# seung-lab/euclidean-distance-transform-3d

Hardware: NVIDIA B200
Metric: Mvoxels/s edtsq 512^3 uint32 (higher is better)
Workload: dtype f32 (u32 labels)

## Files before the change

euclidean-distance-transform-3d_b200/csrc/edt_capi.cu:

```cuda
#include "edt_host.h"
#include "edt_voxel_graph.cuh"
#include "edt_each.cuh"
#include "edt_slab.cuh"

#include <cstdarg>
#include <cstdio>
#include <cstdlib>
#include <cstring>
#include <dlfcn.h>
#include <condition_variable>
#include <functional>
#include <mutex>
#include <thread>
#include <vector>

namespace edtb200 {
namespace host {

thread_local char g_error[512] = "";

int fail(int code, const char* fmt, ...) {
  va_list ap;
  va_start(ap, fmt);
  vsnprintf(g_error, sizeof(g_error), fmt, ap);
// ... 343 lines not shown
    return launch_first<decltype(lw)::Bytes>(labels, f, nlines, sx, wx, border, kflags, dc, s);
  });
}

int later_pass(int axis, int label_bytes, const void* labels, float* f, int64_t sx, int64_t sy, int64_t sz,
               int64_t part, const float* w, int border_lo, int border_hi, int kflags, bool pdl, DeviceCache& dc,
               cudaStream_t s) {
  const int64_t n[2] = {sx, sy};
  const edtb200::LineGeom g = axis == 1 ? geom_for_axis(1, sx, sy, part) : geom_for_axis(2, sx, part, sz);
  return with_label_width(label_bytes, [&](auto lw) {
    return launch_later<decltype(lw)::Bytes>(labels, f, g, w[axis], border_lo, border_hi, kflags, dc, s, pdl,
                                             integer_bound(w, n, axis));
  });
}

template <class T>
cudaError_t grow(T*& p, size_t& have, size_t need) {
  if (have >= need) return cudaSuccess;
  if (p) cudaFree(p);
  p = nullptr; have = 0;
  const cudaError_t e = cudaMalloc(&p, need);
  if (e == cudaSuccess) have = need;
  return e;
}

cudaError_t ensure_stream(cudaStream_t& s) {
  return s ? cudaSuccess : cudaStreamCreateWithFlags(&s, cudaStreamNonBlocking);
}

constexpr int kProfileRing = 256;
thread_local bool g_profile = false;
thread_local cudaEvent_t g_pass_events[kProfileRing][4];
thread_local bool g_pass_events_init = false;
thread_local int g_pass_marks[kProfileRing];
thread_local long g_pass_seq = 0;

void mark_pass(int idx, cudaStream_t stream) {
  if (!g_profile) return;
  if (!g_pass_events_init) {
    for (auto& slot : g_pass_events) for (auto& e : slot) e = nullptr;
    g_pass_events_init = true;
  }
  if (idx == 0) ++g_pass_seq;
  const int slot = (int)((g_pass_seq - 1) % kProfileRing);
  cudaEvent_t& e = g_pass_events[slot][idx];
  if (!e && cudaEventCreate(&e) != cudaSuccess) { cudaGetLastError(); return; }
  cudaEventRecord(e, stream);
  g_pass_marks[slot] = idx;
}

typedef int (*NvtxPushFn)(const char*);
typedef int (*NvtxPopFn)(void);
NvtxPushFn g_nvtx_push = nullptr;
NvtxPopFn g_nvtx_pop = nullptr;
std::once_flag g_nvtx_once;

void nvtx_init() {
  std::call_once(g_nvtx_once, [] {
    if (getenv("EDTB200_NO_NVTX")) return;
    const char* names[] = {"libnvToolsExt.so.1", "libnvToolsExt.so", nullptr};
    for (int i = 0; names[i]; ++i) {
      void* h = dlopen(names[i], RTLD_NOW | RTLD_GLOBAL);
      if (!h) continue;
// ... 5 lines not shown
  });
}
void nvtx_push(const char* name) { nvtx_init(); if (g_nvtx_push) g_nvtx_push(name); }
void nvtx_pop() { if (g_nvtx_pop) g_nvtx_pop(); }

int run_passes(const void* labels, int label_bytes, int ndim, int64_t sx, int64_t sy, int64_t sz,
               float wx, float wy, float wz, int border, int flags, float* f,
               DeviceCache& dc, cudaStream_t stream) {
  const int epilogue = epilogue_flags(flags);
  const float w[3] = {wx, wy, wz};
  int rc = 0;
  static const bool verbose = getenv("EDT_B200_VERBOSE") != nullptr && atoi(getenv("EDT_B200_VERBOSE")) != 0;
  const bool profile_was = g_profile;
  if (verbose) g_profile = true;
  mark_pass(0, stream);
  nvtx_push("edt.x");
  rc = first_pass(label_bytes, labels, f, sy * sz, sx, wx, border,
                  zero_label_flags(flags) | (ndim == 1 ? epilogue : 0), dc, stream);
  nvtx_pop();
  mark_pass(1, stream);
  if (!rc && ndim >= 2) {
    nvtx_push("edt.y");
    rc = later_pass(1, label_bytes, labels, f, sx, sy, sz, sz, w, border, border, ndim == 2 ? epilogue : 0,
                    true, dc, stream);
    nvtx_pop();
    mark_pass(2, stream);
  }
  if (!rc && ndim >= 3) {
    nvtx_push("edt.z");
    rc = later_pass(2, label_bytes, labels, f, sx, sy, sz, sy, w, border, border, epilogue, true, dc,
                    stream);
    nvtx_pop();
    mark_pass(3, stream);
  }
  if (verbose) {
    g_profile = profile_was;
    float ms[3] = {0.0f, 0.0f, 0.0f};
    if (!rc && edtb200_pass_ms(0, ms) == 0) {
      const double nvox = (double)sx * (double)sy * (double)sz;
      const double total = ms[0] + ms[1] + ms[2];
      fprintf(stderr, "[edt_b200] %lldx%lldx%lld L=%d  x %.3f ms  y %.3f ms  z %.3f ms  total %.3f ms  "
                      "%.0f Mvox/s  %.0f GB/s algorithmic\n",
              (long long)sx, (long long)sy, (long long)sz, label_bytes, ms[0], ms[1], ms[2], total,
              total > 0 ? nvox / total / 1e3 : 0.0,
              total > 0 ? nvox * (3.0 * label_bytes + 20.0) / total / 1e6 : 0.0);
    }
  }
  return rc;
}


}

extern "C" {

int edtb200_version(void) { return EDTB200_VERSION; }

const char* edtb200_last_error(void) { return g_error; }
// ... 730 lines not shown
  if (p) { cudaFreeHost(p); cudaGetLastError(); }
}

int edtb200_profile_passes(int enable) {
  g_profile = enable != 0;
  if (enable) g_pass_seq = 0;
  return 0;
}

int edtb200_pass_ms(int steps_back, float* ms3) {
  if (!ms3) return fail(EDTB200_EINVAL, "null pointer");
  ms3[0] = ms3[1] = ms3[2] = 0.0f;
  if (steps_back < 0 || steps_back >= kProfileRing || steps_back >= g_pass_seq)
    return fail(EDTB200_EINVAL, "no profiled transform %d steps back", steps_back);
  const int slot = (int)((g_pass_seq - 1 - steps_back) % kProfileRing);
  for (int i = 0; i < g_pass_marks[slot] && i < 3; ++i) {
    if (!g_pass_events[slot][i] || !g_pass_events[slot][i + 1]) break;
    CUDA_TRY(cudaEventSynchronize(g_pass_events[slot][i + 1]));
    CUDA_TRY(cudaEventElapsedTime(&ms3[i], g_pass_events[slot][i], g_pass_events[slot][i + 1]));
  }
  return 0;
}

int edtb200_release(void) {
  DeviceGuard restore_device;
  int count = 0;
  if (cudaGetDeviceCount(&count) != cudaSuccess) { cudaGetLastError(); return 0; }
  for (int d = 0; d < count && d < kMaxDevices; ++d) {
    DeviceCache& dc = g_cache[d];
    std::lock_guard<std::mutex> host_call(dc.host_call);
    std::lock_guard<std::mutex> guard(dc.lock);
    if (!dc.probed) continue;
    cudaSetDevice(d);
    cudaDeviceSynchronize();
// ... 37 lines not shown
```

euclidean-distance-transform-3d_b200/csrc/edt_host.h:

```cpp
#pragma once
#include "../../include/edt_b200.h"
#include "edt_kernels.cuh"

#include <cstdint>
#include <mutex>

namespace edtb200 {
namespace host {

int fail(int code, const char* fmt, ...);

#define CUDA_TRY(expr)                                                                          \
  do {                                                                                          \
    cudaError_t e__ = (expr);                                                                   \
    if (e__ != cudaSuccess)                                                                     \
      return ::edtb200::host::fail(e__ == cudaErrorMemoryAllocation ? EDTB200_ENOMEM : EDTB200_ECUDA, \
                                   "%s failed: %s", #expr, cudaGetErrorString(e__));            \
  } while (0)

typedef CUresult (*EncodeTiledFn)(CUtensorMap*, CUtensorMapDataType, cuuint32_t, void*, const cuuint64_t*,
                                  const cuuint64_t*, const cuuint32_t*, const cuuint32_t*,
                                  CUtensorMapInterleave, CUtensorMapSwizzle, CUtensorMapL2promotion,
                                  CUtensorMapFloatOOBfill);
EncodeTiledFn tensor_map_encoder();
// ... 17 lines not shown
    cudaEvent_t ready = nullptr; cudaStream_t built_on = nullptr;
    static constexpr int kUsers = 4;
    cudaStream_t user[kUsers] = {nullptr, nullptr, nullptr, nullptr};
    cudaEvent_t used[kUsers] = {nullptr, nullptr, nullptr, nullptr};
    bool user_set[kUsers] = {false, false, false, false};
    bool many_users = false;
  };
  static constexpr int kTables = 16;
  Table tables[kTables];
  uint64_t table_clock = 0;
  cudaMemPool_t pool = nullptr;
  unsigned long long* stat_counter = nullptr;
  unsigned int* stat_ticket = nullptr;
  volatile unsigned long long* stat_publish_host = nullptr;
  unsigned long long* stat_publish_dev = nullptr;
  int sm_count = 0;
  int max_smem_optin = 0;
  bool probed = false;
};

cudaError_t scratch_alloc(DeviceCache& dc, void** p, size_t bytes, cudaStream_t stream);

int step_table(DeviceCache& dc, float w, int count, cudaStream_t stream, const float** out);
int step_table_used(DeviceCache& dc, const float* data, cudaStream_t stream);

template <int Bytes>
int launch_first(const void* labels, float* f, int64_t nlines, int64_t sx, float w, int border, int flags,
                 DeviceCache& dc, cudaStream_t stream);
template <int Bytes>
int launch_later(const void* labels, float* f, const LineGeom& g0, float w, int border_lo, int border_hi,
                 int flags, DeviceCache& dc, cudaStream_t stream, bool pdl, double fmax);

}
}
```

euclidean-distance-transform-3d_b200/csrc/edt_kernels.cuh:

```cuda
#pragma once
#include <cuda.h>
#include <cuda_runtime.h>
#include <math_constants.h>
#include <stdint.h>

namespace edtb200 {

enum : int { kSqrt = 1, kNegate = 2, kZeroLabel = 4 };

constexpr int kNoBoundary = 0x3fffffff;

template <int Bytes> struct LabelOf;
template <> struct LabelOf<1> { using type = uint8_t;  using wide = uint32_t; };
template <> struct LabelOf<2> { using type = uint16_t; using wide = uint32_t; };
template <> struct LabelOf<4> { using type = uint32_t; using wide = uint32_t; };
template <> struct LabelOf<8> { using type = uint64_t; using wide = unsigned long long; };

__device__ __forceinline__ void pdl_launch_dependents() {
  asm volatile("griddepcontrol.launch_dependents;" ::: "memory");
}
__device__ __forceinline__ void pdl_wait_for_previous_grid() {
  asm volatile("griddepcontrol.wait;" ::: "memory");
}

// ... 165 lines not shown
};
template <> struct Vec4Labels<4> {
  static __device__ __forceinline__ void load(const uint32_t* p, uint32_t v[4]) {
    const uint4 w = __ldg(reinterpret_cast<const uint4*>(p));
    v[0] = w.x; v[1] = w.y; v[2] = w.z; v[3] = w.w;
  }
};
template <> struct Vec4Labels<8> {
  static __device__ __forceinline__ void load(const uint64_t* p, unsigned long long v[4]) {
    const ulonglong2 a = __ldg(reinterpret_cast<const ulonglong2*>(p));
    const ulonglong2 b = __ldg(reinterpret_cast<const ulonglong2*>(p) + 1);
    v[0] = a.x; v[1] = a.y; v[2] = b.x; v[3] = b.y;
  }
};

template <int Bytes, int K, bool Plain>
__global__ void __launch_bounds__(256, K >= 8 ? 3 : 5)
first_axis_vec_kernel(const typename LabelOf<Bytes>::type* __restrict__ labels,
                      float* __restrict__ out, int64_t nlines, int sx,
                      const float* __restrict__ table, int border, int flags, RunStat stat) {
  using LT = typename LabelOf<Bytes>::type;
  using WT = typename LabelOf<Bytes>::wide;
  extern __shared__ float table_s[];
  pdl_launch_dependents();
  for (int i = threadIdx.x; i <= sx; i += blockDim.x) table_s[i] = __ldg(table + i);
  if (threadIdx.x == 0) table_s[sx + 1] = __int_as_float(0x7f800000);
  __syncthreads();

  const unsigned full = 0xffffffffu;
  const int lane = threadIdx.x & 31;
  const int warp = threadIdx.x >> 5;
  const int warps = blockDim.x >> 5;
  const unsigned lt_mask = (1u << lane) - 1u;
  const unsigned gt_mask = (lane == 31) ? 0u : (0xfffffffeu << lane);
  const bool keep_background = Plain ? false : (flags & kZeroLabel) != 0;
  unsigned int nstarts = 0;

  for (int64_t line = (int64_t)blockIdx.x * warps + warp; line < nlines;
       line += (int64_t)gridDim.x * warps) {
    const LT* __restrict__ src = labels + line * sx;
    float* __restrict__ dst = out + line * sx;

    WT v[K][4];
#pragma unroll
    for (int b = 0; b < K; ++b) {
      const int q0 = (b << 7) + (lane << 2);
      if (q0 < sx) Vec4Labels<Bytes>::load(src + q0, v[b]);
      else { v[b][0] = v[b][1] = v[b][2] = v[b][3] = 0; }
    }
    uint32_t edges = 0, zeros = 0;
    uint32_t occ[K];
#pragma unroll
    for (int b = 0; b < K; ++b) {
      const int q0 = (b << 7) + (lane << 2);
      WT up = __shfl_up_sync(full, v[b][3], 1);
      if (b > 0) {
        const WT tail = __shfl_sync(full, v[b > 0 ? b - 1 : 0][3], 31);
        if (lane == 0) up = tail;
      }
      uint32_t m = 0, z = 0;
      if (q0 < sx) {
        if ((q0 == 0) ? (border != 0) : (v[b][0] != up)) m |= 1u;
        if (v[b][1] != v[b][0]) m |= 2u;
        if (v[b][2] != v[b][1]) m |= 4u;
        if (v[b][3] != v[b][2]) m |= 8u;
        if (v[b][0] == 0) z |= 1u;
        if (v[b][1] == 0) z |= 2u;
        if (v[b][2] == 0) z |= 4u;
        if (v[b][3] == 0) z |= 8u;
      }
      occ[b] = __ballot_sync(full, m != 0);
      edges |= m << (4 * b);
      zeros |= z << (4 * b);
    }
    nstarts += __popc(edges);

    int kl_in[K], kr_in[K];
    {
      uint32_t prev_occ = 0; int prev_b = 0;
#pragma unroll
      for (int b = 0; b < K; ++b) {
        const int q0 = (b << 7) + (lane << 2);
        const uint32_t mine = occ[b] & lt_mask;
        const uint32_t pick = mine ? mine : prev_occ;
        const int pb = mine ? b : prev_b;
        const int sl = 31 - __clz(pick | 1u);
        const uint32_t nib = (__shfl_sync(full, edges, sl) >> (4 * pb)) & 15u;
        const int pos = (pb << 7) + (sl << 2) + 31 - __clz(nib | 1u);
        kl_in[b] = pick ? (q0 - pos) : kNoBoundary;
        if (occ[b]) { prev_occ = occ[b]; prev_b = b; }
      }
      uint32_t next_occ = 0; int next_b = 0;
#pragma unroll
      for (int b = K - 1; b >= 0; --b) {
        const int q0 = (b << 7) + (lane << 2);
        const uint32_t mine = occ[b] & gt_mask;
        const uint32_t pick = mine ? mine : next_occ;
        const int pb = mine ? b : next_b;
        const int sl = __ffs(pick | 0x80000000u) - 1;
        const uint32_t nib = (__shfl_sync(full, edges, sl) >> (4 * pb)) & 15u;
        const int pos = (pb << 7) + (sl << 2) + __ffs(nib | 8u) - 1;
        const int far = border ? (sx - (q0 + 3)) : kNoBoundary;
        kr_in[b] = pick ? (pos - (q0 + 3)) : far;
        if (occ[b]) { next_occ = occ[b]; next_b = b; }
      }
    }

#pragma unroll
    for (int b = 0; b < K; ++b) {
      const int q0 = (b << 7) + (lane << 2);
      if (q0 >= sx) continue;
      const uint32_t m = (edges >> (4 * b)) & 15u;
      const uint32_t z = (zeros >> (4 * b)) & 15u;
      int kl[4], kr[4];
      int run = kl_in[b];
#pragma unroll
      for (int e = 0; e < 4; ++e) { run = ((m >> e) & 1u) ? 1 : run + 1; kl[e] = run; }
      run = kr_in[b];
      kr[3] = run;
#pragma unroll
      for (int e = 2; e >= 0; --e) { run = ((m >> (e + 1)) & 1u) ? 1 : run + 1; kr[e] = run; }
      float r[4];
#pragma unroll
      for (int e = 0; e < 4; ++e) {
        int k = min(min(kl[e], kr[e]), sx + 1);
        const bool background = (z >> e) & 1u;
        if (background && !keep_background) k = 0;
        float val = table_s[k];
        if (!Plain) val = finish_value(val, background, flags);
        r[e] = val;
      }
      *reinterpret_cast<float4*>(dst + q0) = make_float4(r[0], r[1], r[2], r[3]);
    }
  }
  if (stat.counter) {
#pragma unroll
    for (int s = 16; s > 0; s >>= 1) nstarts += __shfl_xor_sync(full, nstarts, s);
  }
  publish_run_stat(stat, nstarts, lane);
}

struct LineGeom {
  int64_t outer_count;
  int64_t outer_stride;
  int64_t inner_count;
  int64_t line_stride;
  int n;
  int tiles_per_outer;
// ... 26 lines not shown
      : "memory");
  return ok != 0;
}
__device__ __forceinline__ void mbar_wait(uint64_t* bar, unsigned parity) {
  for (unsigned spin = 0; spin < (1u << 26); ++spin)
    if (mbar_try_wait(bar, parity)) return;
  __trap();
}
__device__ __forceinline__ void tma_load_3d(void* dst, const CUtensorMap* map, int c0, int c1, int c2,
                                            uint64_t* bar) {
  asm volatile(
      "cp.async.bulk.tensor.3d.shared::cluster.global.mbarrier::complete_tx::bytes [%0], [%1, {%2, %3, %4}], [%5];"
      ::"r"(smem_addr(dst)), "l"(reinterpret_cast<uint64_t>(map)), "r"(c0), "r"(c1), "r"(c2),
        "r"(smem_addr(bar))
      : "memory");
}

__device__ __forceinline__ float lds_f32(uint32_t addr) {
  float v;
  asm("ld.shared.f32 %0, [%1];" : "=f"(v) : "r"(addr));
  return v;
}
__device__ __forceinline__ uint32_t lds_u32(uint32_t addr) {
  uint32_t v;
  asm("ld.shared.u32 %0, [%1];" : "=r"(v) : "r"(addr));
  return v;
}
__device__ __forceinline__ uint32_t lds_u32_volatile(uint32_t addr) {
  uint32_t v;
  asm volatile("ld.shared.u32 %0, [%1];" : "=r"(v) : "r"(addr) : "memory");
// ... 263 lines not shown
      const float fu = ln.fval(u);
      const float du = (float)(lo - u);
      const float cand = __fmaf_rn(w2f, __fmul_rn(du, du), fu);
      if (!(cand < best)) break;
      best = cand; v = u; fv = fu; dv = du;
    }
    w.v = v; w.fv = fv; w.dv = dv;
    const int wb = (b - 1) >> 5;
    w.wi = v >> 5;
    w.rem = ((v & 31) == 31) ? 0u : (ln.hword(w.wi) & (0xfffffffeu << (v & 31)));
    if (w.wi == wb) w.rem &= 0xffffffffu >> (31 - ((b - 1) & 31));
    walk_advance<TX>(w, ln, lo);
  }
}

template <int Bytes, int TX, bool Epilogue, bool UseTMA, bool Wide, int MinCtas, bool IntHull>
__global__ void __launch_bounds__(Wide ? 1024 : 512, Wide ? 1 : MinCtas)
later_axis_tile_kernel(const __grid_constant__ CUtensorMap fmap,
                       const typename LabelOf<Bytes>::type* __restrict__ labels,
                       float* __restrict__ f, LineGeom g, TileBoxes tb, float w2,
                       int border_lo, int border_hi, int flags, int w2i) {
  using LT = typename LabelOf<Bytes>::type;
  extern __shared__ __align__(128) unsigned char smem_tile[];
  constexpr int SUBS = 32 / TX;
  constexpr bool kRoomy = Wide || MinCtas == 2;
  constexpr bool kDecoupled = Wide;
  constexpr uint32_t ROW = TX * 4;

  const int n = g.n;
  const int nchunks = (n + 31) >> 5;
  const int rows_alloc = UseTMA ? tb.box_rows * tb.nboxes : n;
  const uint32_t fs_a = smem_addr(smem_tile);
  const uint32_t startw_a = fs_a + (uint32_t)rows_alloc * ROW;
  const uint32_t zerow_a = startw_a + (uint32_t)nchunks * ROW;
  const uint32_t hullw_a = zerow_a + (uint32_t)nchunks * ROW;
  const uint32_t sq_a = hullw_a + (uint32_t)nchunks * ROW;
  const uint32_t bar_a = sq_a + (uint32_t)((n + 2 + 1) & ~1) * 4u;
  const uint32_t nz_a = bar_a + 16u;
  const uint32_t cflag_a = nz_a + TX * 4u;
  const bool use_nz = nchunks <= 32;
  uint64_t* bar = reinterpret_cast<uint64_t*>(smem_tile + (bar_a - fs_a));

  const int lane = threadIdx.x & 31;
  const int x = lane & (TX - 1);
  const int chunk0 = (threadIdx.x >> 5) * SUBS + (lane / TX);
  const int chunk_step = (blockDim.x >> 5) * SUBS;

  const int64_t tile = blockIdx.x;
  const int64_t outer = tile / g.tiles_per_outer;
  const int64_t inner0 = (tile - outer * g.tiles_per_outer) * TX;
  const bool live = (inner0 + x) < g.inner_count;
  const LT* __restrict__ tl = labels + (outer * g.outer_stride + inner0);
  float* __restrict__ tf = f + (outer * g.outer_stride + inner0);
  const uint32_t ls = (uint32_t)g.line_stride;
  const size_t pitch = (size_t)ls * sizeof(float);
  const float inf = __int_as_float(0x7f800000);
  const double w2d = (double)w2;

  pdl_launch_dependents();
  if (!UseTMA) pdl_wait_for_previous_grid();
  if (UseTMA && threadIdx.x == 0) {
    if (!kDecoupled) pdl_wait_for_previous_grid();
    mbar_init(bar, 1);
    if (!kDecoupled) {
      mbar_expect_tx(bar, (unsigned)rows_alloc * ROW);
      for (int bx = 0; bx < tb.nboxes; ++bx)
        tma_load_3d(smem_tile + (size_t)bx * tb.box_rows * ROW, &fmap, (int)inner0, bx * tb.box_rows, (int)outer, bar);
    }
  }
  if (threadIdx.x < TX) sts_u32(nz_a + threadIdx.x * 4u, 0u);
  for (int i = threadIdx.x; i < n + 2; i += blockDim.x) {
    const float e = (float)i;
    sts_f32(sq_a + (uint32_t)i * 4u, __fmul_rn(w2, __fmul_rn(e, e)));
  }
  if (kDecoupled) {
    __syncthreads();
    if (UseTMA && threadIdx.x == 0) {
      pdl_wait_for_previous_grid();
      mbar_expect_tx(bar, (unsigned)rows_alloc * ROW);
      for (int bx = 0; bx < tb.nboxes; ++bx)
        tma_load_3d(smem_tile + (size_t)bx * tb.box_rows * ROW, &fmap, (int)inner0, bx * tb.box_rows, (int)outer, bar);
    }
  }

  for (int c = chunk0; c < nchunks; c += chunk_step) {
    const int i0 = c << 5;
    uint32_t wstart = 0, wzero = 0, ext = 1u;
    if (live) {
      uint32_t idx = (uint32_t)i0 * ls + (uint32_t)x;
      const LT* lp = tl + idx;
      LT prev = (i0 > 0) ? tl[idx - ls] : (LT)0;
      uint32_t fdst = fs_a + (uint32_t)i0 * ROW + (uint32_t)x * 4u;
      if (i0 + 32 <= n) {
#pragma unroll
        for (int r = 0; r < 32; ++r) {
          const LT here = kRoomy ? *lp : tl[idx];
          if (kRoomy) lp += ls;
          if (!UseTMA) sts_f32(fdst + r * ROW, tf[idx]);
          if (!UseTMA || !kRoomy) idx += ls;
          if (here != prev) wstart |= (1u << r);
          if (Epilogue && here == 0) wzero |= (1u << r);
          prev = here;
        }
        if (kDecoupled && i0 + 32 < n) ext = (kRoomy ? *lp : tl[idx]) != prev;
      } else {
        for (int r = 0; r < n - i0; ++r) {
          const LT here = kRoomy ? *lp : tl[idx];
          if (kRoomy) lp += ls;
          if (!UseTMA) sts_f32(fdst + r * ROW, tf[idx]);
          if (!UseTMA || !kRoomy) idx += ls;
          if (here != prev) wstart |= (1u << r);
          if (Epilogue && here == 0) wzero |= (1u << r);
          prev = here;
        }
        wstart |= 1u << (n - i0);
      }
      if (i0 == 0) wstart |= 1u;
    }
    sts_u32(startw_a + (uint32_t)c * ROW + (uint32_t)x * 4u, wstart);
    if (Epilogue) sts_u32(zerow_a + (uint32_t)c * ROW + (uint32_t)x * 4u, wzero);
    if (kDecoupled) sts_u8(cflag_a + (uint32_t)(c * TX + x), ext << 2);
  }
  pdl_wait_for_previous_grid();
  if (!UseTMA || !kDecoupled) __syncthreads();
  if (UseTMA) mbar_wait(bar, 0);

  const uint32_t tok = smem_token();
  TileLine<TX> ln;
  ln.f = fs_a + (uint32_t)x * 4u + tok;
  ln.hull = hullw_a + (uint32_t)x * 4u + tok;
  const uint32_t startcol = startw_a + (uint32_t)x * 4u + tok;
  const uint32_t zerocol = zerow_a + (uint32_t)x * 4u + tok;
  const uint32_t sq_t = sq_a + tok;
  const uint32_t cflagcol = cflag_a + (uint32_t)x;
  const uint32_t nzcol = nz_a + (uint32_t)x * 4u;
  char* const line0 = reinterpret_cast<char*>(tf + x);

  int any_cross = 0;
// ... 292 lines not shown
              walk_advance<TX>(w, ln, i);
            }
            w.dv += 1.0f; w.dv1 += 1.0f;
          }
          if (lo_b) best = fminf(best, lds_f32(sq_lo));
          if (hi_b) best = fminf(best, lds_f32(sq_hi));
          if (Epilogue) best = finish_value(best, bg, flags);
          *reinterpret_cast<float*>(dst) = best;
          sq_lo += 4u; sq_hi -= 4u; dst += pitch;
        }
      }
    }
  }
}

__device__ __forceinline__ float parabola_at(float w2, int d, float height) {
  if (d < 4096) {
    const float e = (float)d;
    return __fmaf_rn(w2, __fmul_rn(e, e), height);
  }
  const double e = (double)d;
  return (float)__dadd_rn(__dmul_rn((double)w2, e * e), (double)height);
}

template <int Bytes>
__global__ void __launch_bounds__(128)
later_axis_long_kernel(const typename LabelOf<Bytes>::type* __restrict__ labels,
                       const float* __restrict__ fin, float* __restrict__ fout, int* __restrict__ hull,
                       LineGeom g, float w2, int border_lo, int border_hi, int flags) {
  using LT = typename LabelOf<Bytes>::type;
// ... 135 lines not shown
```

euclidean-distance-transform-3d_b200/csrc/edt_passes.cuh:

```cuda
#pragma once
#include "edt_host.h"

#include <cstdlib>

namespace edtb200 {
namespace host {

inline int env_int(const char* name) { return getenv(name) ? atoi(getenv(name)) : 0; }

struct FirstPlan {
  int vec_k = 0;
  bool epilogue = false;
  size_t smem = 0;
  int block = 0;
  int64_t grid = 0;
};

inline FirstPlan plan_first(int64_t nlines, int64_t sx, int label_bytes, uintptr_t labels_addr, uintptr_t f_addr,
                            int flags, int sm_count, int max_smem_optin, int x_grid) {
  FirstPlan p;
  p.epilogue = flags != 0;
  int64_t cap;
  if (sx % 4 == 0 && sx <= 1024 && labels_addr % (4 * label_bytes) == 0 && f_addr % 16 == 0) {
    p.vec_k = sx <= 128 ? 1 : sx <= 256 ? 2 : sx <= 512 ? 4 : 8;
// ... 139 lines not shown
  }
  if (p.wide) return later_axis_tile_kernel<Bytes, TX, Epi, TMA, true, 3, IH>;
  if constexpr (hot) {
    if (p.ctas == 2) return later_axis_tile_kernel<Bytes, TX, Epi, TMA, false, 2, IH>;
  }
  return later_axis_tile_kernel<Bytes, TX, Epi, TMA, false, 3, IH>;
}

template <int Bytes, int TX = 32>
auto tile_kernel(const LaterPlan& p) {
  if constexpr (TX > 8) {
    if (p.tx < TX) return tile_kernel<Bytes, TX / 2>(p);
  }
  if (p.epilogue) return p.tma ? tile_variant<Bytes, TX, true, true>(p) : tile_variant<Bytes, TX, true, false>(p);
  return p.tma ? tile_variant<Bytes, TX, false, true>(p) : tile_variant<Bytes, TX, false, false>(p);
}

template <int Bytes>
int launch_later(const void* labels, float* f, const LineGeom& g0, float w, int border_lo, int border_hi,
                 int flags, DeviceCache& dc, cudaStream_t stream, bool pdl, double fmax) {
  const auto* lab = static_cast<const typename LabelOf<Bytes>::type*>(labels);
  const float w2 = w * w;
  static const int tile_ctas = env_int("EDTB200_TILE_CTAS");
  static const bool no_pdl = getenv("EDTB200_NO_PDL") != nullptr;
  static const bool no_int_hull = getenv("EDTB200_NO_INT_HULL") != nullptr;
  const bool noise = noise_seen(dc);
  auto plan = [&](bool tma_ok) {
    return plan_later(g0, reinterpret_cast<uintptr_t>(f), w2, flags, fmax, noise, dc.max_smem_optin, tile_ctas,
                      no_int_hull, tma_ok);
  };
// ... 28 lines not shown
  CUDA_TRY(cudaGetLastError());
  CUDA_TRY(cudaMemcpyAsync(f, tmp, bytes, cudaMemcpyDeviceToDevice, stream));
  CUDA_TRY(cudaFreeAsync(hull, stream));
  CUDA_TRY(cudaFreeAsync(tmp, stream));
  return 0;
}

}
}

#define EDT_INSTANTIATE_PASSES(B)                                                                        \
  template int edtb200::host::launch_first<B>(const void*, float*, int64_t, int64_t, float, int, int,    \
                                              edtb200::host::DeviceCache&, cudaStream_t);                \
  template int edtb200::host::launch_later<B>(const void*, float*, const edtb200::LineGeom&, float, int, \
                                              int, int, edtb200::host::DeviceCache&, cudaStream_t, bool, \
                                              double);
```

Before: 238,700.

## Fuse x and y passes into one cluster kernel using distributed shared memory

Adds a fused xy kernel for 3D inputs. Each thread-block cluster covers one z-plane: it computes the x-axis transform, writes it to global memory, and scatters 32-column slices into the shared memory of peer blocks over DSMEM. The y-axis parabola pass then runs from shared memory instead of being a separate kernel launch that reloads f. This removes one launch and one global read of the intermediate f, at the cost of cluster occupancy limits (a non-portable cluster size of 16 for 512 columns) and a fallback path when the cluster does not fit.

```diff
diff --git a/euclidean-distance-transform-3d_b200/csrc/edt_capi.cu b/euclidean-distance-transform-3d_b200/csrc/edt_capi.cu
--- a/euclidean-distance-transform-3d_b200/csrc/edt_capi.cu
+++ b/euclidean-distance-transform-3d_b200/csrc/edt_capi.cu
@@ -381,6 +381,15 @@
   });
 }
 
+int xy_pass(int label_bytes, const void* labels, float* f, int ndim, int64_t sx, int64_t sy, int64_t sz,
+            const float* w, int border, int xflags, DeviceCache& dc, cudaStream_t s, bool* fused) {
+  const int64_t n[2] = {sx, sy};
+  return with_label_width(label_bytes, [&](auto lw) {
+    return launch_xy<decltype(lw)::Bytes>(labels, f, ndim, geom_for_axis(1, sx, sy, sz), sx, w[0], w[1], border,
+                                          xflags, dc, s, integer_bound(w, n, 1), fused);
+  });
+}
+
 template <class T>
 cudaError_t grow(T*& p, size_t& have, size_t need) {
   if (have >= need) return cudaSuccess;
@@ -400,6 +409,7 @@
 thread_local cudaEvent_t g_pass_events[kProfileRing][4];
 thread_local bool g_pass_events_init = false;
 thread_local int g_pass_marks[kProfileRing];
+thread_local bool g_pass_fused[kProfileRing];
 thread_local long g_pass_seq = 0;
 
 void mark_pass(int idx, cudaStream_t stream) {
@@ -414,6 +424,11 @@
   if (!e && cudaEventCreate(&e) != cudaSuccess) { cudaGetLastError(); return; }
   cudaEventRecord(e, stream);
   g_pass_marks[slot] = idx;
+  if (idx == 0) g_pass_fused[slot] = false;
+}
+
+void mark_fused_xy() {
+  if (g_profile && g_pass_seq > 0) g_pass_fused[(g_pass_seq - 1) % kProfileRing] = true;
 }
 
 typedef int (*NvtxPushFn)(const char*);
@@ -449,17 +464,28 @@
   const bool profile_was = g_profile;
   if (verbose) g_profile = true;
   mark_pass(0, stream);
-  nvtx_push("edt.x");
-  rc = first_pass(label_bytes, labels, f, sy * sz, sx, wx, border,
-                  zero_label_flags(flags) | (ndim == 1 ? epilogue : 0), dc, stream);
-  nvtx_pop();
-  mark_pass(1, stream);
+  bool fused = false;
+  if (ndim == 3) {
+    nvtx_push("edt.xy");
+    rc = xy_pass(label_bytes, labels, f, ndim, sx, sy, sz, w, border, zero_label_flags(flags), dc, stream, &fused);
+    nvtx_pop();
+  }
+  if (!rc && !fused) {
+    nvtx_push("edt.x");
+    rc = first_pass(label_bytes, labels, f, sy * sz, sx, wx, border,
+                    zero_label_flags(flags) | (ndim == 1 ? epilogue : 0), dc, stream);
+    nvtx_pop();
+    mark_pass(1, stream);
+  }
   if (!rc && ndim >= 2) {
-    nvtx_push("edt.y");
-    rc = later_pass(1, label_bytes, labels, f, sx, sy, sz, sz, w, border, border, ndim == 2 ? epilogue : 0,
-                    true, dc, stream);
-    nvtx_pop();
+    if (!fused) {
+      nvtx_push("edt.y");
+      rc = later_pass(1, label_bytes, labels, f, sx, sy, sz, sz, w, border, border, ndim == 2 ? epilogue : 0,
+                      true, dc, stream);
+      nvtx_pop();
+    }
     mark_pass(2, stream);
+    if (fused) mark_fused_xy();
   }
   if (!rc && ndim >= 3) {
     nvtx_push("edt.z");
@@ -474,9 +500,11 @@
     if (!rc && edtb200_pass_ms(0, ms) == 0) {
       const double nvox = (double)sx * (double)sy * (double)sz;
       const double total = ms[0] + ms[1] + ms[2];
-      fprintf(stderr, "[edt_b200] %lldx%lldx%lld L=%d  x %.3f ms  y %.3f ms  z %.3f ms  total %.3f ms  "
-                      "%.0f Mvox/s  %.0f GB/s algorithmic\n",
-              (long long)sx, (long long)sy, (long long)sz, label_bytes, ms[0], ms[1], ms[2], total,
+      char passes[96];
+      if (fused) snprintf(passes, sizeof passes, "xy (fused) %.3f ms  z %.3f ms", ms[0] + ms[1], ms[2]);
+      else snprintf(passes, sizeof passes, "x %.3f ms  y %.3f ms  z %.3f ms", ms[0], ms[1], ms[2]);
+      fprintf(stderr, "[edt_b200] %lldx%lldx%lld L=%d  %s  total %.3f ms  %.0f Mvox/s  %.0f GB/s algorithmic\n",
+              (long long)sx, (long long)sy, (long long)sz, label_bytes, passes, total,
               total > 0 ? nvox / total / 1e3 : 0.0,
               total > 0 ? nvox * (3.0 * label_bytes + 20.0) / total / 1e6 : 0.0);
     }
@@ -1237,10 +1265,14 @@
   if (steps_back < 0 || steps_back >= kProfileRing || steps_back >= g_pass_seq)
     return fail(EDTB200_EINVAL, "no profiled transform %d steps back", steps_back);
   const int slot = (int)((g_pass_seq - 1 - steps_back) % kProfileRing);
+  const bool fused = g_pass_fused[slot];
   for (int i = 0; i < g_pass_marks[slot] && i < 3; ++i) {
-    if (!g_pass_events[slot][i] || !g_pass_events[slot][i + 1]) break;
-    CUDA_TRY(cudaEventSynchronize(g_pass_events[slot][i + 1]));
-    CUDA_TRY(cudaEventElapsedTime(&ms3[i], g_pass_events[slot][i], g_pass_events[slot][i + 1]));
+    if (fused && i == 1) continue;
+    const int to = (fused && i == 0) ? 2 : i + 1;
+    if (!g_pass_events[slot][i] || !g_pass_events[slot][to]) break;
+    CUDA_TRY(cudaEventSynchronize(g_pass_events[slot][to]));
+    CUDA_TRY(cudaEventElapsedTime(&ms3[i], g_pass_events[slot][i], g_pass_events[slot][to]));
+    if (fused && i == 0) ms3[1] = ms3[0] = 0.5f * ms3[0];
   }
   return 0;
 }
diff --git a/euclidean-distance-transform-3d_b200/csrc/edt_host.h b/euclidean-distance-transform-3d_b200/csrc/edt_host.h
--- a/euclidean-distance-transform-3d_b200/csrc/edt_host.h
+++ b/euclidean-distance-transform-3d_b200/csrc/edt_host.h
@@ -55,6 +55,10 @@
   unsigned int* stat_ticket = nullptr;
   volatile unsigned long long* stat_publish_host = nullptr;
   unsigned long long* stat_publish_dev = nullptr;
+  struct ClusterFit { const void* kern = nullptr; int size = 0; int threads = 0; size_t smem = 0; int clusters = 0; };
+  static constexpr int kClusterFits = 8;
+  ClusterFit cluster_fits[kClusterFits];
+  unsigned cluster_fit_next = 0;
   int sm_count = 0;
   int max_smem_optin = 0;
   bool probed = false;
@@ -71,6 +75,9 @@
 template <int Bytes>
 int launch_later(const void* labels, float* f, const LineGeom& g0, float w, int border_lo, int border_hi,
                  int flags, DeviceCache& dc, cudaStream_t stream, bool pdl, double fmax);
+template <int Bytes>
+int launch_xy(const void* labels, float* f, int ndim, const LineGeom& g, int64_t sx, float wx, float wy,
+              int border, int xflags, DeviceCache& dc, cudaStream_t stream, double fmax, bool* fused);
 
 }
 }
diff --git a/euclidean-distance-transform-3d_b200/csrc/edt_kernels.cuh b/euclidean-distance-transform-3d_b200/csrc/edt_kernels.cuh
--- a/euclidean-distance-transform-3d_b200/csrc/edt_kernels.cuh
+++ b/euclidean-distance-transform-3d_b200/csrc/edt_kernels.cuh
@@ -203,13 +203,112 @@
   }
 };
 
+template <int Bytes, int K, bool Plain, class Store>
+__device__ __forceinline__ void first_axis_vec_line(const typename LabelOf<Bytes>::type* __restrict__ src, int sx,
+                                                    const float* table_s, int border, int flags, bool keep_background,
+                                                    int lane, unsigned lt_mask, unsigned gt_mask,
+                                                    unsigned int& nstarts, Store store) {
+  using WT = typename LabelOf<Bytes>::wide;
+  const unsigned full = 0xffffffffu;
+  WT v[K][4];
+#pragma unroll
+  for (int b = 0; b < K; ++b) {
+    const int q0 = (b << 7) + (lane << 2);
+    if (q0 < sx) Vec4Labels<Bytes>::load(src + q0, v[b]);
+    else { v[b][0] = v[b][1] = v[b][2] = v[b][3] = 0; }
+  }
+  uint32_t edges = 0, zeros = 0;
+  uint32_t occ[K];
+#pragma unroll
+  for (int b = 0; b < K; ++b) {
+    const int q0 = (b << 7) + (lane << 2);
+    WT up = __shfl_up_sync(full, v[b][3], 1);
+    if (b > 0) {
+      const WT tail = __shfl_sync(full, v[b > 0 ? b - 1 : 0][3], 31);
+      if (lane == 0) up = tail;
+    }
+    uint32_t m = 0, z = 0;
+    if (q0 < sx) {
+      if ((q0 == 0) ? (border != 0) : (v[b][0] != up)) m |= 1u;
+      if (v[b][1] != v[b][0]) m |= 2u;
+      if (v[b][2] != v[b][1]) m |= 4u;
+      if (v[b][3] != v[b][2]) m |= 8u;
+      if (v[b][0] == 0) z |= 1u;
+      if (v[b][1] == 0) z |= 2u;
+      if (v[b][2] == 0) z |= 4u;
+      if (v[b][3] == 0) z |= 8u;
+    }
+    occ[b] = __ballot_sync(full, m != 0);
+    edges |= m << (4 * b);
+    zeros |= z << (4 * b);
+  }
+  nstarts += __popc(edges);
+
+  int kl_in[K], kr_in[K];
+  {
+    uint32_t prev_occ = 0; int prev_b = 0;
+#pragma unroll
+    for (int b = 0; b < K; ++b) {
+      const int q0 = (b << 7) + (lane << 2);
+      const uint32_t mine = occ[b] & lt_mask;
+      const uint32_t pick = mine ? mine : prev_occ;
+      const int pb = mine ? b : prev_b;
+      const int sl = 31 - __clz(pick | 1u);
+      const uint32_t nib = (__shfl_sync(full, edges, sl) >> (4 * pb)) & 15u;
+      const int pos = (pb << 7) + (sl << 2) + 31 - __clz(nib | 1u);
+      kl_in[b] = pick ? (q0 - pos) : kNoBoundary;
+      if (occ[b]) { prev_occ = occ[b]; prev_b = b; }
+    }
+    uint32_t next_occ = 0; int next_b = 0;
+#pragma unroll
+    for (int b = K - 1; b >= 0; --b) {
+      const int q0 = (b << 7) + (lane << 2);
+      const uint32_t mine = occ[b] & gt_mask;
+      const uint32_t pick = mine ? mine : next_occ;
+      const int pb = mine ? b : next_b;
+      const int sl = __ffs(pick | 0x80000000u) - 1;
+      const uint32_t nib = (__shfl_sync(full, edges, sl) >> (4 * pb)) & 15u;
+      const int pos = (pb << 7) + (sl << 2) + __ffs(nib | 8u) - 1;
+      const int far = border ? (sx - (q0 + 3)) : kNoBoundary;
+      kr_in[b] = pick ? (pos - (q0 + 3)) : far;
+      if (occ[b]) { next_occ = occ[b]; next_b = b; }
+    }
+  }
+
+#pragma unroll
+  for (int b = 0; b < K; ++b) {
+    const int q0 = (b << 7) + (lane << 2);
+    if (q0 >= sx) continue;
+    const uint32_t m = (edges >> (4 * b)) & 15u;
+    const uint32_t z = (zeros >> (4 * b)) & 15u;
+    int kl[4], kr[4];
+    int run = kl_in[b];
+#pragma unroll
+    for (int e = 0; e < 4; ++e) { run = ((m >> e) & 1u) ? 1 : run + 1; kl[e] = run; }
+    run = kr_in[b];
+    kr[3] = run;
+#pragma unroll
+    for (int e = 2; e >= 0; --e) { run = ((m >> (e + 1)) & 1u) ? 1 : run + 1; kr[e] = run; }
+    float r[4];
+#pragma unroll
+    for (int e = 0; e < 4; ++e) {
+      int k = min(min(kl[e], kr[e]), sx + 1);
+      const bool background = (z >> e) & 1u;
+      if (background && !keep_background) k = 0;
+      float val = table_s[k];
+      if (!Plain) val = finish_value(val, background, flags);
+      r[e] = val;
+    }
+    store(q0, make_float4(r[0], r[1], r[2], r[3]));
+  }
+}
+
 template <int Bytes, int K, bool Plain>
 __global__ void __launch_bounds__(256, K >= 8 ? 3 : 5)
 first_axis_vec_kernel(const typename LabelOf<Bytes>::type* __restrict__ labels,
                       float* __restrict__ out, int64_t nlines, int sx,
                       const float* __restrict__ table, int border, int flags, RunStat stat) {
   using LT = typename LabelOf<Bytes>::type;
-  using WT = typename LabelOf<Bytes>::wide;
   extern __shared__ float table_s[];
   pdl_launch_dependents();
   for (int i = threadIdx.x; i <= sx; i += blockDim.x) table_s[i] = __ldg(table + i);
@@ -229,98 +328,8 @@
        line += (int64_t)gridDim.x * warps) {
     const LT* __restrict__ src = labels + line * sx;
     float* __restrict__ dst = out + line * sx;
-
-    WT v[K][4];
-#pragma unroll
-    for (int b = 0; b < K; ++b) {
-      const int q0 = (b << 7) + (lane << 2);
-      if (q0 < sx) Vec4Labels<Bytes>::load(src + q0, v[b]);
-      else { v[b][0] = v[b][1] = v[b][2] = v[b][3] = 0; }
-    }
-    uint32_t edges = 0, zeros = 0;
-    uint32_t occ[K];
-#pragma unroll
-    for (int b = 0; b < K; ++b) {
-      const int q0 = (b << 7) + (lane << 2);
-      WT up = __shfl_up_sync(full, v[b][3], 1);
-      if (b > 0) {
-        const WT tail = __shfl_sync(full, v[b > 0 ? b - 1 : 0][3], 31);
-        if (lane == 0) up = tail;
-      }
-      uint32_t m = 0, z = 0;
-      if (q0 < sx) {
-        if ((q0 == 0) ? (border != 0) : (v[b][0] != up)) m |= 1u;
-        if (v[b][1] != v[b][0]) m |= 2u;
-        if (v[b][2] != v[b][1]) m |= 4u;
-        if (v[b][3] != v[b][2]) m |= 8u;
-        if (v[b][0] == 0) z |= 1u;
-        if (v[b][1] == 0) z |= 2u;
-        if (v[b][2] == 0) z |= 4u;
-        if (v[b][3] == 0) z |= 8u;
-      }
-      occ[b] = __ballot_sync(full, m != 0);
-      edges |= m << (4 * b);
-      zeros |= z << (4 * b);
-    }
-    nstarts += __popc(edges);
-
-    int kl_in[K], kr_in[K];
-    {
-      uint32_t prev_occ = 0; int prev_b = 0;
-#pragma unroll
-      for (int b = 0; b < K; ++b) {
-        const int q0 = (b << 7) + (lane << 2);
-        const uint32_t mine = occ[b] & lt_mask;
-        const uint32_t pick = mine ? mine : prev_occ;
-        const int pb = mine ? b : prev_b;
-        const int sl = 31 - __clz(pick | 1u);
-        const uint32_t nib = (__shfl_sync(full, edges, sl) >> (4 * pb)) & 15u;
-        const int pos = (pb << 7) + (sl << 2) + 31 - __clz(nib | 1u);
-        kl_in[b] = pick ? (q0 - pos) : kNoBoundary;
-        if (occ[b]) { prev_occ = occ[b]; prev_b = b; }
-      }
-      uint32_t next_occ = 0; int next_b = 0;
-#pragma unroll
-      for (int b = K - 1; b >= 0; --b) {
-        const int q0 = (b << 7) + (lane << 2);
-        const uint32_t mine = occ[b] & gt_mask;
-        const uint32_t pick = mine ? mine : next_occ;
-        const int pb = mine ? b : next_b;
-        const int sl = __ffs(pick | 0x80000000u) - 1;
-        const uint32_t nib = (__shfl_sync(full, edges, sl) >> (4 * pb)) & 15u;
-        const int pos = (pb << 7) + (sl << 2) + __ffs(nib | 8u) - 1;
-        const int far = border ? (sx - (q0 + 3)) : kNoBoundary;
-        kr_in[b] = pick ? (pos - (q0 + 3)) : far;
-        if (occ[b]) { next_occ = occ[b]; next_b = b; }
-      }
-    }
-
-#pragma unroll
-    for (int b = 0; b < K; ++b) {
-      const int q0 = (b << 7) + (lane << 2);
-      if (q0 >= sx) continue;
-      const uint32_t m = (edges >> (4 * b)) & 15u;
-      const uint32_t z = (zeros >> (4 * b)) & 15u;
-      int kl[4], kr[4];
-      int run = kl_in[b];
-#pragma unroll
-      for (int e = 0; e < 4; ++e) { run = ((m >> e) & 1u) ? 1 : run + 1; kl[e] = run; }
-      run = kr_in[b];
-      kr[3] = run;
-#pragma unroll
-      for (int e = 2; e >= 0; --e) { run = ((m >> (e + 1)) & 1u) ? 1 : run + 1; kr[e] = run; }
-      float r[4];
-#pragma unroll
-      for (int e = 0; e < 4; ++e) {
-        int k = min(min(kl[e], kr[e]), sx + 1);
-        const bool background = (z >> e) & 1u;
-        if (background && !keep_background) k = 0;
-        float val = table_s[k];
-        if (!Plain) val = finish_value(val, background, flags);
-        r[e] = val;
-      }
-      *reinterpret_cast<float4*>(dst + q0) = make_float4(r[0], r[1], r[2], r[3]);
-    }
+    first_axis_vec_line<Bytes, K, Plain>(src, sx, table_s, border, flags, keep_background, lane, lt_mask, gt_mask,
+                                         nstarts, [&](int q0, float4 r) { *reinterpret_cast<float4*>(dst + q0) = r; });
   }
   if (stat.counter) {
 #pragma unroll
@@ -377,6 +386,23 @@
       ::"r"(smem_addr(dst)), "l"(reinterpret_cast<uint64_t>(map)), "r"(c0), "r"(c1), "r"(c2),
         "r"(smem_addr(bar))
       : "memory");
+}
+
+__device__ __forceinline__ void cluster_arrive_relaxed() {
+  asm volatile("barrier.cluster.arrive.relaxed.aligned;" ::: "memory");
+}
+__device__ __forceinline__ void cluster_arrive_release() {
+  asm volatile("barrier.cluster.arrive.release.aligned;" ::: "memory");
+}
+__device__ __forceinline__ void cluster_wait_acquire() {
+  asm volatile("barrier.cluster.wait.acquire.aligned;" ::: "memory");
+}
+__device__ __forceinline__ void st_cluster_f32x4(uint32_t addr, uint32_t rank, float4 v) {
+  uint32_t remote;
+  asm volatile("mapa.shared::cluster.u32 %0, %1, %2;" : "=r"(remote) : "r"(addr), "r"(rank));
+  asm volatile("st.shared::cluster.v4.f32 [%0], {%1, %2, %3, %4};" ::"r"(remote), "f"(v.x), "f"(v.y), "f"(v.z),
+               "f"(v.w)
+               : "memory");
 }
 
 __device__ __forceinline__ float lds_f32(uint32_t addr) {
@@ -670,13 +696,16 @@
   }
 }
 
-template <int Bytes, int TX, bool Epilogue, bool UseTMA, bool Wide, int MinCtas, bool IntHull>
-__global__ void __launch_bounds__(Wide ? 1024 : 512, Wide ? 1 : MinCtas)
-later_axis_tile_kernel(const __grid_constant__ CUtensorMap fmap,
-                       const typename LabelOf<Bytes>::type* __restrict__ labels,
-                       float* __restrict__ f, LineGeom g, TileBoxes tb, float w2,
-                       int border_lo, int border_hi, int flags, int w2i) {
+enum : int { kStagePlain = 0, kStageTMA = 1, kStageCluster = 2 };
+
+template <int Bytes, int TX, bool Epilogue, int Staging, bool Wide, int MinCtas, bool IntHull>
+__device__ __forceinline__ void tile_pass(const CUtensorMap* fmap, const typename LabelOf<Bytes>::type* __restrict__ labels,
+                                          float* __restrict__ f, LineGeom g, TileBoxes tb, float w2,
+                                          int border_lo, int border_hi, int flags, int w2i,
+                                          unsigned tid, unsigned nthreads) {
   using LT = typename LabelOf<Bytes>::type;
+  constexpr bool UseTMA = Staging == kStageTMA;
+  constexpr bool LoadF = Staging == kStagePlain;
   extern __shared__ __align__(128) unsigned char smem_tile[];
   constexpr int SUBS = 32 / TX;
   constexpr bool kRoomy = Wide || MinCtas == 2;
@@ -697,10 +726,10 @@
   const bool use_nz = nchunks <= 32;
   uint64_t* bar = reinterpret_cast<uint64_t*>(smem_tile + (bar_a - fs_a));
 
-  const int lane = threadIdx.x & 31;
+  const int lane = tid & 31;
   const int x = lane & (TX - 1);
-  const int chunk0 = (threadIdx.x >> 5) * SUBS + (lane / TX);
-  const int chunk_step = (blockDim.x >> 5) * SUBS;
+  const int chunk0 = (tid >> 5) * SUBS + (lane / TX);
+  const int chunk_step = (nthreads >> 5) * SUBS;
 
   const int64_t tile = blockIdx.x;
   const int64_t outer = tile / g.tiles_per_outer;
@@ -713,29 +742,29 @@
   const float inf = __int_as_float(0x7f800000);
   const double w2d = (double)w2;
 
-  pdl_launch_dependents();
-  if (!UseTMA) pdl_wait_for_previous_grid();
-  if (UseTMA && threadIdx.x == 0) {
+  if (Staging != kStageCluster) pdl_launch_dependents();
+  if (LoadF) pdl_wait_for_previous_grid();
+  if (UseTMA && tid == 0) {
     if (!kDecoupled) pdl_wait_for_previous_grid();
     mbar_init(bar, 1);
     if (!kDecoupled) {
       mbar_expect_tx(bar, (unsigned)rows_alloc * ROW);
       for (int bx = 0; bx < tb.nboxes; ++bx)
-        tma_load_3d(smem_tile + (size_t)bx * tb.box_rows * ROW, &fmap, (int)inner0, bx * tb.box_rows, (int)outer, bar);
-    }
-  }
-  if (threadIdx.x < TX) sts_u32(nz_a + threadIdx.x * 4u, 0u);
-  for (int i = threadIdx.x; i < n + 2; i += blockDim.x) {
+        tma_load_3d(smem_tile + (size_t)bx * tb.box_rows * ROW, fmap, (int)inner0, bx * tb.box_rows, (int)outer, bar);
+    }
+  }
+  if (tid < TX) sts_u32(nz_a + tid * 4u, 0u);
+  for (int i = tid; i < n + 2; i += nthreads) {
     const float e = (float)i;
     sts_f32(sq_a + (uint32_t)i * 4u, __fmul_rn(w2, __fmul_rn(e, e)));
   }
   if (kDecoupled) {
     __syncthreads();
-    if (UseTMA && threadIdx.x == 0) {
+    if (UseTMA && tid == 0) {
       pdl_wait_for_previous_grid();
       mbar_expect_tx(bar, (unsigned)rows_alloc * ROW);
       for (int bx = 0; bx < tb.nboxes; ++bx)
-        tma_load_3d(smem_tile + (size_t)bx * tb.box_rows * ROW, &fmap, (int)inner0, bx * tb.box_rows, (int)outer, bar);
+        tma_load_3d(smem_tile + (size_t)bx * tb.box_rows * ROW, fmap, (int)inner0, bx * tb.box_rows, (int)outer, bar);
     }
   }
 
@@ -752,8 +781,8 @@
         for (int r = 0; r < 32; ++r) {
           const LT here = kRoomy ? *lp : tl[idx];
           if (kRoomy) lp += ls;
-          if (!UseTMA) sts_f32(fdst + r * ROW, tf[idx]);
-          if (!UseTMA || !kRoomy) idx += ls;
+          if (LoadF) sts_f32(fdst + r * ROW, tf[idx]);
+          if (LoadF || !kRoomy) idx += ls;
           if (here != prev) wstart |= (1u << r);
           if (Epilogue && here == 0) wzero |= (1u << r);
           prev = here;
@@ -763,8 +792,8 @@
         for (int r = 0; r < n - i0; ++r) {
           const LT here = kRoomy ? *lp : tl[idx];
           if (kRoomy) lp += ls;
-          if (!UseTMA) sts_f32(fdst + r * ROW, tf[idx]);
-          if (!UseTMA || !kRoomy) idx += ls;
+          if (LoadF) sts_f32(fdst + r * ROW, tf[idx]);
+          if (LoadF || !kRoomy) idx += ls;
           if (here != prev) wstart |= (1u << r);
           if (Epilogue && here == 0) wzero |= (1u << r);
           prev = here;
@@ -777,7 +806,8 @@
     if (Epilogue) sts_u32(zerow_a + (uint32_t)c * ROW + (uint32_t)x * 4u, wzero);
     if (kDecoupled) sts_u8(cflag_a + (uint32_t)(c * TX + x), ext << 2);
   }
-  pdl_wait_for_previous_grid();
+  if (Staging == kStageCluster) cluster_wait_acquire();
+  else pdl_wait_for_previous_grid();
   if (!UseTMA || !kDecoupled) __syncthreads();
   if (UseTMA) mbar_wait(bar, 0);
 
@@ -1100,6 +1130,63 @@
   }
 }
 
+template <int Bytes, int TX, bool Epilogue, bool UseTMA, bool Wide, int MinCtas, bool IntHull>
+__global__ void __launch_bounds__(Wide ? 1024 : 512, Wide ? 1 : MinCtas)
+later_axis_tile_kernel(const __grid_constant__ CUtensorMap fmap,
+                       const typename LabelOf<Bytes>::type* __restrict__ labels,
+                       float* __restrict__ f, LineGeom g, TileBoxes tb, float w2,
+                       int border_lo, int border_hi, int flags, int w2i) {
+  tile_pass<Bytes, TX, Epilogue, UseTMA ? kStageTMA : kStagePlain, Wide, MinCtas, IntHull>(
+      &fmap, labels, f, g, tb, w2, border_lo, border_hi, flags, w2i, threadIdx.x, blockDim.x);
+}
+
+template <int Bytes, int MinCtas, bool IntHull>
+__global__ void __launch_bounds__(512, MinCtas)
+xy_cluster_kernel(const typename LabelOf<Bytes>::type* __restrict__ labels, float* __restrict__ f, LineGeom g,
+                  int sx, const float* __restrict__ table, int border, int xflags, RunStat stat, float w2, int w2i) {
+  extern __shared__ __align__(128) unsigned char smem_tile[];
+  pdl_launch_dependents();
+  cluster_arrive_relaxed();
+  const int n = g.n;
+  const int c_count = g.tiles_per_outer;
+  const int rank = (int)(blockIdx.x % (unsigned)c_count);
+  const int64_t plane = blockIdx.x / (unsigned)c_count;
+  const uint32_t fs_a = smem_addr(smem_tile);
+  float* table_s = reinterpret_cast<float*>(smem_tile + (size_t)n * 128);
+  for (int i = threadIdx.x; i <= sx; i += blockDim.x) table_s[i] = __ldg(table + i);
+  if (threadIdx.x == 0) table_s[sx + 1] = __int_as_float(0x7f800000);
+  __syncthreads();
+  cluster_wait_acquire();
+
+  const int lane = threadIdx.x & 31;
+  const int warps = blockDim.x >> 5;
+  const unsigned lt_mask = (1u << lane) - 1u;
+  const unsigned gt_mask = (lane == 31) ? 0u : (0xfffffffeu << lane);
+  const bool keep_background = (xflags & kZeroLabel) != 0;
+  const int rows = (n + c_count - 1) / c_count;
+  const int y1 = min(n, (rank + 1) * rows);
+  unsigned int nstarts = 0;
+  for (int y = rank * rows + (threadIdx.x >> 5); y < y1; y += warps) {
+    const int64_t line = plane * n + y;
+    float* __restrict__ dst = f + line * sx;
+    const uint32_t row_a = fs_a + (uint32_t)y * 128u;
+    first_axis_vec_line<Bytes, 4, false>(labels + line * sx, sx, table_s, border, xflags, keep_background, lane,
+                                         lt_mask, gt_mask, nstarts, [&](int q0, float4 r) {
+      *reinterpret_cast<float4*>(dst + q0) = r;
+      st_cluster_f32x4(row_a + (uint32_t)(q0 & 31) * 4u, (uint32_t)(q0 >> 5), r);
+    });
+  }
+  if (stat.counter) {
+#pragma unroll
+    for (int s = 16; s > 0; s >>= 1) nstarts += __shfl_xor_sync(0xffffffffu, nstarts, s);
+  }
+  publish_run_stat(stat, nstarts, lane);
+  __syncthreads();
+  cluster_arrive_release();
+  tile_pass<Bytes, 32, false, kStageCluster, false, MinCtas, IntHull>(nullptr, labels, f, g, TileBoxes{0, 0}, w2,
+                                                                      border, border, 0, w2i, threadIdx.x, blockDim.x);
+}
+
 __device__ __forceinline__ float parabola_at(float w2, int d, float height) {
   if (d < 4096) {
     const float e = (float)d;
diff --git a/euclidean-distance-transform-3d_b200/csrc/edt_passes.cuh b/euclidean-distance-transform-3d_b200/csrc/edt_passes.cuh
--- a/euclidean-distance-transform-3d_b200/csrc/edt_passes.cuh
+++ b/euclidean-distance-transform-3d_b200/csrc/edt_passes.cuh
@@ -177,6 +177,101 @@
   }
   if (p.epilogue) return p.tma ? tile_variant<Bytes, TX, true, true>(p) : tile_variant<Bytes, TX, true, false>(p);
   return p.tma ? tile_variant<Bytes, TX, false, true>(p) : tile_variant<Bytes, TX, false, false>(p);
+}
+
+struct XyPlan {
+  bool fused = false;
+  int clusters = 0;
+  int ctas = 3;
+  bool int_hull = false;
+  size_t smem = 0;
+  int threads = 0;
+  int64_t grid = 0;
+  LineGeom g;
+};
+
+inline XyPlan plan_xy(int ndim, const LineGeom& g, int64_t sx, int label_bytes, uintptr_t labels_addr,
+                      uintptr_t f_addr, float w2, double fmax, bool noise_hint, int max_smem_optin, int tile_ctas,
+                      bool no_int_hull) {
+  XyPlan p;
+  if (ndim != 3 || sx > 512 || sx % 4 != 0 || labels_addr % (4 * label_bytes) != 0 || f_addr % 16 != 0) return p;
+  const LaterPlan y = plan_later(g, f_addr, w2, 0, fmax, noise_hint, max_smem_optin, tile_ctas, no_int_hull, true);
+  if (!y.tile || y.tx != 32 || !y.tma || y.wide) return p;
+  p.clusters = (int)((sx + 31) / 32);
+  p.ctas = y.ctas;
+  p.int_hull = y.int_hull;
+  const size_t fs = (size_t)g.n * 32 * 4;
+  p.smem = tile_smem_bytes(g.n, 32, g.n);
+  if (fs + sizeof(float) * (size_t)(sx + 2) > p.smem) p.smem = fs + sizeof(float) * (size_t)(sx + 2);
+  if (p.smem > (size_t)max_smem_optin) return p;
+  p.threads = y.warps * 32;
+  p.g = g;
+  p.g.tiles_per_outer = p.clusters;
+  p.grid = (int64_t)p.clusters * g.outer_count;
+  p.fused = p.grid <= 0x7fffffffLL;
+  return p;
+}
+
+template <int Bytes>
+auto xy_kernel(const XyPlan& p) {
+  if (p.ctas == 2) return p.int_hull ? xy_cluster_kernel<Bytes, 2, true> : xy_cluster_kernel<Bytes, 2, false>;
+  return p.int_hull ? xy_cluster_kernel<Bytes, 3, true> : xy_cluster_kernel<Bytes, 3, false>;
+}
+
+template <int Bytes>
+int launch_xy(const void* labels, float* f, int ndim, const LineGeom& g, int64_t sx, float wx, float wy,
+              int border, int xflags, DeviceCache& dc, cudaStream_t stream, double fmax, bool* fused) {
+  *fused = false;
+  static const bool no_fused = getenv("EDTB200_NO_FUSED_XY") != nullptr;
+  static const int tile_ctas = env_int("EDTB200_TILE_CTAS");
+  static const bool no_int_hull = getenv("EDTB200_NO_INT_HULL") != nullptr;
+  if (no_fused) return 0;
+  const float w2 = wy * wy;
+  const XyPlan p = plan_xy(ndim, g, sx, Bytes, reinterpret_cast<uintptr_t>(labels), reinterpret_cast<uintptr_t>(f),
+                           w2, fmax, noise_seen(dc), dc.max_smem_optin, tile_ctas, no_int_hull);
+  if (!p.fused) return 0;
+  const auto kern = xy_kernel<Bytes>(p);
+  cudaLaunchAttribute attr;
+  attr.id = cudaLaunchAttributeClusterDimension;
+  attr.val.clusterDim.x = (unsigned)p.clusters;
+  attr.val.clusterDim.y = 1;
+  attr.val.clusterDim.z = 1;
+  const cudaLaunchConfig_t cfg = {dim3((unsigned)p.grid), dim3((unsigned)p.threads), p.smem, stream, &attr, 1u};
+  int clusters = 0;
+  {
+    std::lock_guard<std::mutex> hold(dc.lock);
+    auto& fits = dc.cluster_fits;
+    int i = 0;
+    while (i < DeviceCache::kClusterFits && !(fits[i].kern == (const void*)kern && fits[i].size == p.clusters &&
+                                             fits[i].threads == p.threads && fits[i].smem == p.smem))
+      ++i;
+    if (i < DeviceCache::kClusterFits) {
+      clusters = fits[i].clusters;
+    } else {
+      CUDA_TRY(cudaFuncSetAttribute(kern, cudaFuncAttributeNonPortableClusterSizeAllowed, 1));
+      CUDA_TRY(cudaFuncSetAttribute(kern, cudaFuncAttributeMaxDynamicSharedMemorySize, (int)p.smem));
+      if (cudaOccupancyMaxActiveClusters(&clusters, kern, &cfg) != cudaSuccess) {
+        cudaGetLastError();
+        clusters = 0;
+      }
+      auto& slot = fits[dc.cluster_fit_next++ % DeviceCache::kClusterFits];
+      slot.kern = (const void*)kern; slot.size = p.clusters; slot.threads = p.threads; slot.smem = p.smem;
+      slot.clusters = clusters;
+    }
+  }
+  if (clusters <= 0) return 0;
+
+  const float* table = nullptr;
+  int trc = step_table(dc, wx, (int)sx + 1, stream, &table);
+  if (trc) return trc;
+  const RunStat stat = {dc.stat_counter, dc.stat_ticket, dc.stat_publish_dev,
+                        (unsigned long long)(g.n * g.outer_count) * (unsigned long long)sx};
+  CUDA_TRY(cudaFuncSetAttribute(kern, cudaFuncAttributeMaxDynamicSharedMemorySize, (int)p.smem));
+  CUDA_TRY(cudaLaunchKernelEx(&cfg, kern, static_cast<const typename LabelOf<Bytes>::type*>(labels), f, p.g,
+                              (int)sx, table, border, xflags, stat, w2, p.int_hull ? (int)w2 : 0));
+  CUDA_TRY(cudaGetLastError());
+  *fused = true;
+  return step_table_used(dc, table, stream);
 }
 
 template <int Bytes>
@@ -235,4 +330,7 @@
                                               edtb200::host::DeviceCache&, cudaStream_t);                \
   template int edtb200::host::launch_later<B>(const void*, float*, const edtb200::LineGeom&, float, int, \
                                               int, int, edtb200::host::DeviceCache&, cudaStream_t, bool, \
-                                              double);
+                                              double);                                                   \
+  template int edtb200::host::launch_xy<B>(const void*, float*, int, const edtb200::LineGeom&, int64_t,  \
+                                           float, float, int, int, edtb200::host::DeviceCache&,          \
+                                           cudaStream_t, double, bool*);
```

Result: slower. 179,400 (median of 6 runs) (-24.8%).
